# NVlabs/neuralrgbd

Measured on AMD Instinct MI355X. Metric: depth frames/sec @256x192x64cand, 5-view window; warp-kernel HBM GB/s vs peak, higher is better.
Workload: dtype f32; 1 GPU; plane-sweep grid 256x192x64cand (image 1024x768); config_id=B, depth_candidates=64, views=5, streams_per_gpu=1, streams_total=1, parallelism=replicas x1 (independent video streams)

## Files before the change

### neuralrgbd_amd/csrc/wino_dw4.hip

```cpp
#include "wino_dw.hpp"

namespace nrgbd {

constexpr int kD4ScratchWave = 8 * 64 * 4;

__device__ __forceinline__ int d4_t(int p) { return p < 4 ? p + 1 : (p == 4 ? 0 : 5); }
__device__ __forceinline__ int d4_nslot(int t) { return (t == 0 || t == 5) ? 3 : 4; }
__device__ __forceinline__ int d4_j(int t, int k) {
    if (t == 0) return k == 0 ? 4 : (k == 1 ? 0 : 2);
    if (t == 5) return k == 0 ? 5 : (k == 1 ? 1 : 3);
    return k == 0 ? 4 : k;
}
__device__ __forceinline__ float d4_c(int t, int k) {
    if (k == 0) return 1.f;
    if (t == 0 || t == 5) return k == 1 ? 0.5625f : -2.5f;
    const float s = (t & 1) ? -1.f : 1.f;
    if (t <= 2) return k == 1 ? s * 1.125f : (k == 2 ? -2.25f : -s * 0.5f);
    return k == 1 ? s * 0.375f : (k == 2 ? -0.25f : -s * 1.5f);
}

struct WinoD4Args {
    WinoPcArgs b;
    float* scratch;
};

struct D4Stash { f32x4* A; f32x4* B; __amdgpu_buffer_rsrc_t C; int laneC; };

template <int P>
__device__ __forceinline__ void d4_fold(const DwAcc& acc, const WinoPcArgs& a, const DwLane& c, const DwTile& tl, int wv, const D4Stash& st, f32x2 n1) {
    constexpr int NEMIT = P == 3 ? 2 : (P >= 4 ? 1 : 0);
    constexpr int ZS0 = P == 3 ? 1 : (P == 4 ? 0 : 3);
    f32x2 S1[NEMIT ? NEMIT : 1] = {}, S2[NEMIT ? NEMIT : 1] = {};
    float* ybase = a.y + (((size_t)tl.z0 * a.H + tl.y0) * a.W + tl.x0) * a.Cout + tl.cg * 64 + wv * 16;
    const size_t zstride = (size_t)a.H * a.W * a.Cout;
#pragma unroll
    for (int m = 0; m < 2; ++m) {
#pragma unroll
        for (int rp = 0; rp < 2; ++rp) {
            f32x2 tr[2][4];
            dw_plane_inverse(acc, m, rp, n1, tr);
#pragma unroll
            for (int aa = 0; aa < 2; ++aa) {
                const int wi = (m * 2 + rp) * 2 + aa;
                const f32x4 o = dw_plane_word(tr, aa, n1);
                if constexpr (P == 0) {
                    st.A[wi * 64] = o;
                } else if constexpr (P == 1) {
                    const f32x4 m1v = st.A[wi * 64];
                    st.A[wi * 64] = m1v + o;
                    st.B[wi * 64] = m1v - o;
                } else if constexpr (P == 2) {
                    __builtin_amdgcn_raw_buffer_store_b128(__builtin_bit_cast(i32x4_t, o), st.C, st.laneC, wi * 1024, 0);
                } else if constexpr (P == 3) {
                    const f32x4 m3v = __builtin_bit_cast(f32x4, __builtin_amdgcn_raw_buffer_load_b128(st.C, st.laneC, wi * 1024, 0));
                    {
                        const f32x4 d34 = m3v - o, d12 = st.B[wi * 64];
                        st.B[wi * 64] = 0.125f * d12 + 3.375f * d34;
                        dw_emit(a, c, ybase + 1 * zstride, m, rp, aa, 0.5f * d12 + 1.5f * d34, S1[0], S2[0]);
                    }
                    __builtin_amdgcn_sched_barrier(0);
                    {
                        const f32x4 s34 = m3v + o, s12 = st.A[wi * 64];
                        st.A[wi * 64] = s12 + s34;
                        dw_emit(a, c, ybase + 2 * zstride, m, rp, aa, 0.25f * s12 + 2.25f * s34, S1[1], S2[1]);
                    }
                    __builtin_amdgcn_sched_barrier(0);
                } else if constexpr (P == 4) {
                    dw_emit(a, c, ybase, m, rp, aa, st.A[wi * 64] + o, S1[0], S2[0]);
                } else {
                    dw_emit(a, c, ybase + 3 * zstride, m, rp, aa, st.B[wi * 64] + o, S1[0], S2[0]);
                }
            }
            __builtin_amdgcn_sched_barrier(0);
        }
    }
    if constexpr (NEMIT >= 1) dw_store_stats(a, c, tl.cg * 64 + wv * 16 + c.jj, tl.row0 + ZS0, S1, S2);
}

struct D4Regs { f32x4 pre[kDwNPF]; };

__device__ __forceinline__ void d4_issue(const WinoPcArgs& a, const DwProd& P, bool nx, int j, int cb, D4Regs& r) {
    const int tz = (nx ? P.tn.z0 : P.tl.z0) - 1 + j;
    const int z = __builtin_amdgcn_readfirstlane(min(max(tz, 0), a.N - 1));
    const size_t base = ((size_t)z * P.plane + (size_t)(__builtin_amdgcn_readfirstlane(cb) * kCB)) * sizeof(float);
    const __amdgpu_buffer_rsrc_t xb = pc_rsrc(reinterpret_cast<const char*>(a.x) + base);
#pragma unroll
    for (int u = 0; u < kDwNPF; ++u) r.pre[u] = pc_bload(xb, nx ? P.nxt.off[u] : P.cur.off[u]);
}

template <bool IDENT, bool CLAMP>
__device__ __forceinline__ void d4_combine(const WinoPcArgs& a, const DwProd& P, int NS, int ncb, int s, int p, int cbi, D4Regs& set0, D4Regs& set1,
                                           D4Regs& set2, D4Regs& set3) {
    float* raw = P.strip(P.gi & 1);
    const int t = d4_t(p), cb = dw_cb(p, cbi, ncb), nsl = d4_nslot(t);
    const bool nx = s + 1 >= NS;
    const int cbn = cbi + 1 == ncb ? 0 : cbi + 1, pn = nx ? 0 : (cbi + 1 == ncb ? p + 1 : p);
    const int tnx = d4_t(pn), cbne = dw_cb(pn, cbn, ncb);
    f32x4 ssw[2] = {{1.f, 1.f, 0.f, 0.f}, {1.f, 1.f, 0.f, 0.f}};
    if constexpr (!IDENT) {
        ssw[0] = *reinterpret_cast<const f32x4*>(P.ssl + 2 * (cb * kCB + P.p.w4 * 4));
        ssw[1] = *reinterpret_cast<const f32x4*>(P.ssl + 2 * (cb * kCB + P.p.w4 * 4) + 4);
    }
    const int nsn = d4_nslot(tnx);
    float c[4];
#pragma unroll
    for (int k = 0; k < 4; ++k) {
        const int z = P.tl.z0 - 1 + d4_j(t, k < nsl ? k : 0);
        c[k] = (k < nsl && z >= 0 && z < a.N) ? d4_c(t, k) : 0.f;
    }
    f32x2 lo[kDwNPF], hi[kDwNPF], ul[kDwNPF], uh[kDwNPF];
    dw_activate<IDENT, CLAMP>(set0.pre, ssw, a.x_relu, ul, uh);
    if (c[0] != 0.f) {
#pragma unroll
        for (int i = 0; i < kDwNPF; ++i) { lo[i] = ul[i]; hi[i] = uh[i]; }
    } else {
#pragma unroll
        for (int i = 0; i < kDwNPF; ++i) { lo[i] = f32x2{0.f, 0.f}; hi[i] = f32x2{0.f, 0.f}; }
    }
    d4_issue(a, P, nx && P.has_next, d4_j(tnx, 0), cbne, set0);
    dw_activate<IDENT, CLAMP>(set1.pre, ssw, a.x_relu, ul, uh);
    {
        const f32x2 c1 = {c[1], c[1]};
#pragma unroll
        for (int i = 0; i < kDwNPF; ++i) { lo[i] = __builtin_elementwise_fma(ul[i], c1, lo[i]); hi[i] = __builtin_elementwise_fma(uh[i], c1, hi[i]); }
    }
    d4_issue(a, P, nx && P.has_next, d4_j(tnx, 1), cbne, set1);
    dw_activate<IDENT, CLAMP>(set2.pre, ssw, a.x_relu, ul, uh);
    {
        const f32x2 c2 = {c[2], c[2]};
#pragma unroll
        for (int i = 0; i < kDwNPF; ++i) { lo[i] = __builtin_elementwise_fma(ul[i], c2, lo[i]); hi[i] = __builtin_elementwise_fma(uh[i], c2, hi[i]); }
    }
    d4_issue(a, P, nx && P.has_next, d4_j(tnx, 2), cbne, set2);
    if (nsl > 3) {
        dw_activate<IDENT, CLAMP>(set3.pre, ssw, a.x_relu, ul, uh);
        const f32x2 c3 = {c[3], c[3]};
#pragma unroll
        for (int i = 0; i < kDwNPF; ++i) { lo[i] = __builtin_elementwise_fma(ul[i], c3, lo[i]); hi[i] = __builtin_elementwise_fma(uh[i], c3, hi[i]); }
    }
    if (nsn > 3) d4_issue(a, P, nx && P.has_next, d4_j(tnx, 3), cbne, set3);
#pragma unroll
    for (int i = 0; i < kDwNPF; ++i) {
        if (!P.interior) {
            const f32x2 kk = {P.cur.keep[i], P.cur.keep[i]};
            lo[i] = lo[i] * kk; hi[i] = hi[i] * kk;
        }
        *reinterpret_cast<f32x4*>(raw + P.p.wr_off[i]) = __builtin_shufflevector(lo[i], hi[i], 0, 1, 2, 3);
    }
}

template <bool IDENT, bool CLAMP>
__global__ __launch_bounds__(512) void conv_wino_dw4_kernel(const WinoD4Args aa) {
    const WinoPcArgs& a = aa.b;
    extern __shared__ __attribute__((aligned(16))) float lds[];
    float* Vb = lds;
    float* rawb = lds + kDwNBuf * kPcV;
    float* stashb = rawb + kDwStrips;
    float* ssl = stashb + 4 * kDwStashWave;

    const int tid = threadIdx.x, lane = tid & 63;
    const int wave = __builtin_amdgcn_readfirstlane(tid >> 6);
    const int wv = wave & 3;
    const int ncb = a.Cin / kCB;
    const int NS = 6 * ncb;

    int first, step, end;
    pc_tile_share(a.ntiles, first, step, end);
    if (first >= end) return;
    const int count = (end - first + step - 1) / step;
    pc_load_ss_table<false>(ssl, a.Cin, a.x_ss, nullptr, CLAMP ? a.x_unit : 1.f);
    __syncthreads();

    if (wave >= 4) {
        const DwLane c = dw_lane(a, lane, wv);
        DwAcc acc;
        const size_t wgroup = (size_t)NS * 16 * 256;
        D4Stash st;
        st.A = reinterpret_cast<f32x4*>(stashb + wv * kDwStashWave) + lane;
        st.B = st.A + 8 * 64;
        st.C = pc_rsrc(reinterpret_cast<const char*>(aa.scratch) + ((size_t)blockIdx.x * 4 + wv) * kD4ScratchWave * sizeof(float));
        st.laneC = lane * 16;
        DwTile tl = dw_decode<4>(first, a);
        const f32x4* wt = c.wbase + (size_t)tl.cg * wgroup;
        f32x4 Bn[kPcNB], An[2][2];
        const f32x2 n1 = dw_prime(Bn, An, wt, Vb, c);
        int buf = 0;
        for (int it = 0; it < count; ++it) {
            const int tnext = first + (it + 1 < count ? it + 1 : it) * step;
            const DwTile tn = dw_decode<4>(tnext, a);
            const f32x4* wt_next = c.wbase + (size_t)tn.cg * wgroup;
            dw_phase<0, 6>(acc, An, Bn, Vb, buf, wt, wt_next, ncb, c);
            d4_fold<0>(acc, a, c, tl, wv, st, n1);
            dw_phase<1, 6>(acc, An, Bn, Vb, buf, wt, wt_next, ncb, c);
            d4_fold<1>(acc, a, c, tl, wv, st, n1);
            dw_phase<2, 6>(acc, An, Bn, Vb, buf, wt, wt_next, ncb, c);
            d4_fold<2>(acc, a, c, tl, wv, st, n1);
            dw_phase<3, 6>(acc, An, Bn, Vb, buf, wt, wt_next, ncb, c);
            d4_fold<3>(acc, a, c, tl, wv, st, n1);
            dw_phase<4, 6>(acc, An, Bn, Vb, buf, wt, wt_next, ncb, c);
            d4_fold<4>(acc, a, c, tl, wv, st, n1);
            dw_phase<5, 6>(acc, An, Bn, Vb, buf, wt, wt_next, ncb, c);
            d4_fold<5>(acc, a, c, tl, wv, st, n1);
            tl = tn;
            wt = wt_next;
        }
    } else {
        DwProd P;
        dw_prod_init<4, false>(a, P, wv, lane, Vb, rawb, ssl, first);
        D4Regs set0, set1, set2, set3;
        {
            const int t0 = d4_t(0), cb0 = dw_cb(0, 0, ncb);
            d4_issue(a, P, false, d4_j(t0, 0), cb0, set0);
            d4_issue(a, P, false, d4_j(t0, 1), cb0, set1);
            d4_issue(a, P, false, d4_j(t0, 2), cb0, set2);
            d4_issue(a, P, false, d4_j(t0, 3 < d4_nslot(t0) ? 3 : 0), cb0, set3);
        }
        for (int it = 0; it < count; ++it) {
            dw_tile_begin(a, P, it + 1 < count);
            int cbi = 0, p = 0;
            for (int s = 0; s < NS; ++s) {
                if (s == NS - 1 && P.has_next) dw_next_tile<4, false>(a, P, first + (it + 1) * step);
                d4_combine<IDENT, CLAMP>(a, P, NS, ncb, s, p, cbi, set0, set1, set2, set3);
                if (P.gi > 0) dw_transform(P.p, P.strip((P.gi & 1) ^ 1), Vb + P.qbuf * kPcV);
                __syncthreads();
                dw_stage_end(P);
                if (++cbi == ncb) { cbi = 0; ++p; }
            }
            dw_tile_end(P);
        }
        dw_transform(P.p, P.strip((P.gi & 1) ^ 1), Vb + P.qbuf * kPcV);
        __syncthreads();
        __syncthreads();
    }
}

}

extern "C" int nrgbd_conv_wino_dw4_pack(const float* w, float* w_wino, int Cin, int Cout, int transposed, void* stream) {
    return nrgbd::dw_pack<6>(w, w_wino, Cin, Cout, transposed, stream);
}

extern "C" int nrgbd_conv_wino_dw4_workspace(int N, int H, int W, int Cout, size_t* bytes) {
    if (!bytes) return NRGBD_E_NULL;
    if (N <= 0 || (N & 3) || H <= 0 || W <= 0 || Cout <= 0 || Cout % 64) return NRGBD_E_SHAPE;
    int n = 0;
    const int rc = nrgbd::dw_workgroups(4, N, H, W, Cout, &n);
    if (rc != NRGBD_OK) return rc;
    *bytes = (size_t)n * 4 * nrgbd::kD4ScratchWave * sizeof(float);
    return NRGBD_OK;
}

extern "C" int nrgbd_conv_wino_dw4_f32(const float* x, const float* x_ss, int x_relu, float x_unit, const float* w_wino, float* y,
                                       float* stats, void* workspace, size_t workspace_bytes, int N, int H, int W, int Cin, int Cout,
                                       void* stream) {
    using namespace nrgbd;
    if (!x || !w_wino || !y || !workspace) return NRGBD_E_NULL;
    int rows = 0, nwg = 0;
    long nt = 0;
    int rc = dw_check(4, N, H, W, Cin, Cout, &rows, &nt);
    if (rc != NRGBD_OK) return rc;
    if (reinterpret_cast<uintptr_t>(workspace) & 15) return NRGBD_E_ALIGN;
    const bool clamp = x_unit != 0.f;
    if (clamp && (!x_ss || !x_relu || !dw_unit_ok(x_unit))) return NRGBD_E_ARG;
    if (nt >= (1L << 31)) return NRGBD_E_SHAPE;
    rc = dw_workgroups(4, N, H, W, Cout, &nwg);
    if (rc != NRGBD_OK) return rc;
    if (workspace_bytes < (size_t)nwg * 4 * kD4ScratchWave * sizeof(float)) return NRGBD_E_NULL;
    WinoD4Args aa{};
    aa.b = WinoPcArgs{x, x_ss, nullptr, nullptr, nullptr, w_wino, y, stats, x_relu, 0, N, H, W, Cin, Cout, (int)nt, rows,
                      nullptr, 0, 0, 0, 0, x_unit};
    aa.scratch = static_cast<float*>(workspace);
    const DwLaunch l{nwg, dw_lds_bytes(1, Cin), dw_lds_attr(1), (hipStream_t)stream};
    if (clamp) return dw_launch<conv_wino_dw4_kernel<false, true>>(l, aa);
    if (!x_ss && !x_relu) return dw_launch<conv_wino_dw4_kernel<true, false>>(l, aa);
    return dw_launch<conv_wino_dw4_kernel<false, false>>(l, aa);
}
```

Baseline: 30.86 frames/s.

## Pair Winograd input-transform rows to reuse loaded depth slices across phases

For small channel counts (ncb<=4), the producer computes the odd transform row alongside the even one from the same loaded depth slices. The odd row's results are kept in registers, one kept set per channel block, and written out in the following phase instead of being reloaded and recomputed. This is meant to cut global loads and activation work for phases 0-3, at the cost of many extra live VGPRs. The prefetch schedule becomes more intricate, and the cross-phase register keeping risks spills or lower occupancy. It also depends on the channel-block ordering being identity in the paired phases.

```diff
diff --git a/neuralrgbd_amd/csrc/wino_dw4.hip b/neuralrgbd_amd/csrc/wino_dw4.hip
--- a/neuralrgbd_amd/csrc/wino_dw4.hip
+++ b/neuralrgbd_amd/csrc/wino_dw4.hip
@@ -78,6 +78,31 @@
 }
 
 struct D4Regs { f32x4 pre[kDwNPF]; };
+struct D4Keep { f32x2 lo[kDwNPF], hi[kDwNPF]; };
+
+template <bool PAIR>
+__device__ __forceinline__ void d4_chain(const f32x2 (&ul)[kDwNPF], const f32x2 (&uh)[kDwNPF], float c, float cp, f32x2 (&lo)[kDwNPF],
+                                         f32x2 (&hi)[kDwNPF], D4Keep& kp) {
+    const f32x2 c2 = {c, c};
+#pragma unroll
+    for (int i = 0; i < kDwNPF; ++i) { lo[i] = __builtin_elementwise_fma(ul[i], c2, lo[i]); hi[i] = __builtin_elementwise_fma(uh[i], c2, hi[i]); }
+    if constexpr (PAIR) {
+        const f32x2 p2 = {cp, cp};
+#pragma unroll
+        for (int i = 0; i < kDwNPF; ++i) { kp.lo[i] = __builtin_elementwise_fma(ul[i], p2, kp.lo[i]); kp.hi[i] = __builtin_elementwise_fma(uh[i], p2, kp.hi[i]); }
+    }
+}
+
+__device__ __forceinline__ void d4_mask(const DwProd& P, f32x2 (&lo)[kDwNPF], f32x2 (&hi)[kDwNPF]) {
+    if (!P.interior) {
+        asm volatile("");
+#pragma unroll
+        for (int i = 0; i < kDwNPF; ++i) {
+            const f32x2 kk = {P.cur.keep[i], P.cur.keep[i]};
+            lo[i] = lo[i] * kk; hi[i] = hi[i] * kk;
+        }
+    }
+}
 
 __device__ __forceinline__ void d4_issue(const WinoPcArgs& a, const DwProd& P, bool nx, int j, int cb, D4Regs& r) {
     const int tz = (nx ? P.tn.z0 : P.tl.z0) - 1 + j;
@@ -88,64 +113,109 @@
     for (int u = 0; u < kDwNPF; ++u) r.pre[u] = pc_bload(xb, nx ? P.nxt.off[u] : P.cur.off[u]);
 }
 
-template <bool IDENT, bool CLAMP>
+template <bool IDENT, bool CLAMP, bool PAIR>
 __device__ __forceinline__ void d4_combine(const WinoPcArgs& a, const DwProd& P, int NS, int ncb, int s, int p, int cbi, D4Regs& set0, D4Regs& set1,
-                                           D4Regs& set2, D4Regs& set3) {
+                                           D4Regs& set2, D4Regs& set3, D4Keep& kp) {
     float* raw = P.strip(P.gi & 1);
-    const int t = d4_t(p), cb = dw_cb(p, cbi, ncb), nsl = d4_nslot(t);
-    const bool nx = s + 1 >= NS;
+    const int t = d4_t(p), cb = PAIR ? cbi : dw_cb(p, cbi, ncb), nsl = d4_nslot(t);
+    const bool nx = !PAIR && s + 1 >= NS;
+    const bool refill = !PAIR || cbi + 1 < ncb;
     const int cbn = cbi + 1 == ncb ? 0 : cbi + 1, pn = nx ? 0 : (cbi + 1 == ncb ? p + 1 : p);
-    const int tnx = d4_t(pn), cbne = dw_cb(pn, cbn, ncb);
+    const int tnx = PAIR ? t : d4_t(pn), cbne = PAIR ? cbi + 1 : dw_cb(pn, cbn, ncb);
     f32x4 ssw[2] = {{1.f, 1.f, 0.f, 0.f}, {1.f, 1.f, 0.f, 0.f}};
     if constexpr (!IDENT) {
         ssw[0] = *reinterpret_cast<const f32x4*>(P.ssl + 2 * (cb * kCB + P.p.w4 * 4));
         ssw[1] = *reinterpret_cast<const f32x4*>(P.ssl + 2 * (cb * kCB + P.p.w4 * 4) + 4);
     }
     const int nsn = d4_nslot(tnx);
-    float c[4];
+    float c[4], cp[4];
 #pragma unroll
     for (int k = 0; k < 4; ++k) {
         const int z = P.tl.z0 - 1 + d4_j(t, k < nsl ? k : 0);
-        c[k] = (k < nsl && z >= 0 && z < a.N) ? d4_c(t, k) : 0.f;
+        const bool in = k < nsl && z >= 0 && z < a.N;
+        c[k] = in ? d4_c(t, k) : 0.f;
+        cp[k] = PAIR && in ? d4_c(t + 1, k) : 0.f;
     }
     f32x2 lo[kDwNPF], hi[kDwNPF], ul[kDwNPF], uh[kDwNPF];
-    dw_activate<IDENT, CLAMP>(set0.pre, ssw, a.x_relu, ul, uh);
-    if (c[0] != 0.f) {
-#pragma unroll
-        for (int i = 0; i < kDwNPF; ++i) { lo[i] = ul[i]; hi[i] = uh[i]; }
-    } else {
+    dw_activate<IDENT, CLAMP>(set0.pre, ssw, a.x_relu, lo, hi);
+    if (c[0] == 0.f) {
+        asm volatile("");
 #pragma unroll
         for (int i = 0; i < kDwNPF; ++i) { lo[i] = f32x2{0.f, 0.f}; hi[i] = f32x2{0.f, 0.f}; }
     }
-    d4_issue(a, P, nx && P.has_next, d4_j(tnx, 0), cbne, set0);
+    if constexpr (PAIR) {
+#pragma unroll
+        for (int i = 0; i < kDwNPF; ++i) { kp.lo[i] = lo[i]; kp.hi[i] = hi[i]; }
+    }
+    if (refill) d4_issue(a, P, nx && P.has_next, d4_j(tnx, 0), cbne, set0);
     dw_activate<IDENT, CLAMP>(set1.pre, ssw, a.x_relu, ul, uh);
-    {
-        const f32x2 c1 = {c[1], c[1]};
-#pragma unroll
-        for (int i = 0; i < kDwNPF; ++i) { lo[i] = __builtin_elementwise_fma(ul[i], c1, lo[i]); hi[i] = __builtin_elementwise_fma(uh[i], c1, hi[i]); }
-    }
-    d4_issue(a, P, nx && P.has_next, d4_j(tnx, 1), cbne, set1);
+    d4_chain<PAIR>(ul, uh, c[1], cp[1], lo, hi, kp);
+    if (refill) d4_issue(a, P, nx && P.has_next, d4_j(tnx, 1), cbne, set1);
     dw_activate<IDENT, CLAMP>(set2.pre, ssw, a.x_relu, ul, uh);
-    {
-        const f32x2 c2 = {c[2], c[2]};
-#pragma unroll
-        for (int i = 0; i < kDwNPF; ++i) { lo[i] = __builtin_elementwise_fma(ul[i], c2, lo[i]); hi[i] = __builtin_elementwise_fma(uh[i], c2, hi[i]); }
-    }
-    d4_issue(a, P, nx && P.has_next, d4_j(tnx, 2), cbne, set2);
+    d4_chain<PAIR>(ul, uh, c[2], cp[2], lo, hi, kp);
+    if (refill) d4_issue(a, P, nx && P.has_next, d4_j(tnx, 2), cbne, set2);
     if (nsl > 3) {
         dw_activate<IDENT, CLAMP>(set3.pre, ssw, a.x_relu, ul, uh);
-        const f32x2 c3 = {c[3], c[3]};
-#pragma unroll
-        for (int i = 0; i < kDwNPF; ++i) { lo[i] = __builtin_elementwise_fma(ul[i], c3, lo[i]); hi[i] = __builtin_elementwise_fma(uh[i], c3, hi[i]); }
-    }
-    if (nsn > 3) d4_issue(a, P, nx && P.has_next, d4_j(tnx, 3), cbne, set3);
+        d4_chain<PAIR>(ul, uh, c[3], cp[3], lo, hi, kp);
+    }
+    if (refill && nsn > 3) d4_issue(a, P, nx && P.has_next, d4_j(tnx, 3), cbne, set3);
+    d4_mask(P, lo, hi);
+#pragma unroll
+    for (int i = 0; i < kDwNPF; ++i) *reinterpret_cast<f32x4*>(raw + P.p.wr_off[i]) = __builtin_shufflevector(lo[i], hi[i], 0, 1, 2, 3);
+}
+
+__device__ __forceinline__ void d4_restore(const WinoPcArgs& a, const DwProd& P, int ncb, int p, int cbi, const D4Keep& kp, D4Regs& set0,
+                                           D4Regs& set1, D4Regs& set2, D4Regs& set3) {
+    float* raw = P.strip(P.gi & 1);
+    const int tnx = d4_t(p + 1), cbne = 0, nsn = d4_nslot(tnx);
+    const int k0 = 4 * cbi / ncb, k1 = 4 * (cbi + 1) / ncb;
+    f32x2 lo[kDwNPF], hi[kDwNPF];
+#pragma unroll
+    for (int i = 0; i < kDwNPF; ++i) { lo[i] = kp.lo[i]; hi[i] = kp.hi[i]; }
+    d4_mask(P, lo, hi);
+    if (k0 <= 0 && 0 < k1) d4_issue(a, P, false, d4_j(tnx, 0), cbne, set0);
+    *reinterpret_cast<f32x4*>(raw + P.p.wr_off[0]) = __builtin_shufflevector(lo[0], hi[0], 0, 1, 2, 3);
+    if (k0 <= 1 && 1 < k1) d4_issue(a, P, false, d4_j(tnx, 1), cbne, set1);
+    *reinterpret_cast<f32x4*>(raw + P.p.wr_off[1]) = __builtin_shufflevector(lo[1], hi[1], 0, 1, 2, 3);
+    if (k0 <= 2 && 2 < k1) d4_issue(a, P, false, d4_j(tnx, 2), cbne, set2);
+    *reinterpret_cast<f32x4*>(raw + P.p.wr_off[2]) = __builtin_shufflevector(lo[2], hi[2], 0, 1, 2, 3);
+    if (k0 <= 3 && 3 < k1 && nsn > 3) d4_issue(a, P, false, d4_j(tnx, 3), cbne, set3);
+}
+
+template <int SET>
+__device__ __forceinline__ void d4_keep(D4Keep& k, const D4Keep& v) {
 #pragma unroll
     for (int i = 0; i < kDwNPF; ++i) {
-        if (!P.interior) {
-            const f32x2 kk = {P.cur.keep[i], P.cur.keep[i]};
-            lo[i] = lo[i] * kk; hi[i] = hi[i] * kk;
-        }
-        *reinterpret_cast<f32x4*>(raw + P.p.wr_off[i]) = __builtin_shufflevector(lo[i], hi[i], 0, 1, 2, 3);
+        asm volatile("v_mov_b64 %0, %1 ; keep set %2" : "+v"(k.lo[i]) : "v"(v.lo[i]), "n"(SET));
+        asm volatile("v_mov_b64 %0, %1 ; keep set %2" : "+v"(k.hi[i]) : "v"(v.hi[i]), "n"(SET));
+    }
+}
+template <int SET>
+__device__ __forceinline__ void d4_restore_set(const WinoPcArgs& a, const DwProd& P, int ncb, int p, int cbi, const D4Keep& k, D4Regs& set0,
+                                               D4Regs& set1, D4Regs& set2, D4Regs& set3) {
+    asm volatile("; kept set %0" ::"n"(SET));
+    d4_restore(a, P, ncb, p, cbi, k, set0, set1, set2, set3);
+    asm volatile("; kept set %0 written" ::"n"(SET));
+}
+
+template <bool IDENT, bool CLAMP>
+__device__ __forceinline__ void d4_stage(const WinoPcArgs& a, const DwProd& P, bool pair, int NS, int ncb, int s, int p, int cbi, D4Regs& set0,
+                                         D4Regs& set1, D4Regs& set2, D4Regs& set3, D4Keep& k0, D4Keep& k1, D4Keep& k2, D4Keep& k3) {
+    const int cb = dw_cb(p, cbi, ncb);
+    D4Keep kp;
+    if (!pair || p >= 4) {
+        d4_combine<IDENT, CLAMP, false>(a, P, NS, ncb, s, p, cbi, set0, set1, set2, set3, kp);
+    } else if (!(p & 1)) {
+        d4_combine<IDENT, CLAMP, true>(a, P, NS, ncb, s, p, cbi, set0, set1, set2, set3, kp);
+        if (cb == 0) d4_keep<0>(k0, kp);
+        else if (cb == 1) d4_keep<1>(k1, kp);
+        else if (cb == 2) d4_keep<2>(k2, kp);
+        else d4_keep<3>(k3, kp);
+    } else {
+        if (cb == 0) d4_restore_set<0>(a, P, ncb, p, cbi, k0, set0, set1, set2, set3);
+        else if (cb == 1) d4_restore_set<1>(a, P, ncb, p, cbi, k1, set0, set1, set2, set3);
+        else if (cb == 2) d4_restore_set<2>(a, P, ncb, p, cbi, k2, set0, set1, set2, set3);
+        else d4_restore_set<3>(a, P, ncb, p, cbi, k3, set0, set1, set2, set3);
     }
 }
 
@@ -215,12 +285,14 @@
             d4_issue(a, P, false, d4_j(t0, 2), cb0, set2);
             d4_issue(a, P, false, d4_j(t0, 3 < d4_nslot(t0) ? 3 : 0), cb0, set3);
         }
+        const bool pair = ncb <= 4;
+        D4Keep k0 = {}, k1 = {}, k2 = {}, k3 = {};
         for (int it = 0; it < count; ++it) {
             dw_tile_begin(a, P, it + 1 < count);
             int cbi = 0, p = 0;
             for (int s = 0; s < NS; ++s) {
                 if (s == NS - 1 && P.has_next) dw_next_tile<4, false>(a, P, first + (it + 1) * step);
-                d4_combine<IDENT, CLAMP>(a, P, NS, ncb, s, p, cbi, set0, set1, set2, set3);
+                d4_stage<IDENT, CLAMP>(a, P, pair, NS, ncb, s, p, cbi, set0, set1, set2, set3, k0, k1, k2, k3);
                 if (P.gi > 0) dw_transform(P.p, P.strip((P.gi & 1) ^ 1), Vb + P.qbuf * kPcV);
                 __syncthreads();
                 dw_stage_end(P);
```

Result: faster. 31.39 frames/s (median of 6 runs) (+1.7%).
